# ChenyuWang-Monica/REED

Measured on AMD Instinct MI355X. Metric: SiT-XL/2 ImageNet-256 train images/sec, higher is better.
Workload: dtype bf16

## Files before the change

### include/reed_hip.h

```cpp
#ifndef REED_HIP_H
#define REED_HIP_H
#include <stdint.h>
#ifdef __cplusplus
extern "C" {
#endif

const char* reed_last_error(void);
int reed_version(void);
int reed_half_kind(void);

int reed_gemm(int layout, int epilogue, const void* P, int64_t ldp, const void* Q, int64_t ldq,
              int M, int N, int K, void* C, int64_t ldc, void* C2, int64_t ldc2, const void* R,
              int64_t ldr, const void* bias, const void* gate, int64_t ldgate, int rows_per_gate,
              float* dbias, int accumulate, int split_k, int64_t slab_stride, void* stream);

int reed_wgrad_group(int n, const void* const* dy, const void* const* x, float* const* dw, float* const* dbias,
                     const int* n_out, const int* k_in, int tokens, int accumulate, void* stream);
int reed_wgrad_group_deal(int n, const int* n_out, const int* k_in, const int* has_bias, int cus, unsigned* items);

int reed_set_cu_reserve(int n);
int reed_planning_cus(void);
int reed_set_concurrent_comm(int on);

int reed_gemm_force_tile(int tile);

int64_t reed_colsum_ws_floats(int M, int N);
int reed_colsum_bf16(const void* x, int64_t ld, float* ws, float* out, int M, int N, int accumulate,
                     void* stream);

int reed_reduce_slabs(const float* slabs, int64_t stride, int nslabs, float* out, int64_t n,
                      int accumulate, void* stream);

int reed_ln_modulate_fwd(const float* x, const void* shift, const void* scale, int64_t ldmod,
                         void* h, float* mean, float* rstd, int M, int D, int T, float eps,
                         void* stream);
int reed_ln_modulate_bwd(const void* dh, const float* x, const float* mean, const float* rstd,
                         const void* scale, int64_t ldmod, float* dx, float* part, int M, int D,
                         int T, void* stream);

int reed_ln_modulate_bwd_gate(const void* dh, const float* x, const float* mean, const float* rstd,
                              const void* scale, int64_t ldmod, float* dx, float* part, const void* y,
                              const void* gate, int64_t ldgate, void* dy, float* part_g, float* part_dy,
                              int M, int D, int T, void* stream);

int reed_gate_bwd(const float* dx, const void* y, const void* gate, int64_t ldgate, void* dy,
                  float* part, float* part_dy, int M, int D, int T, void* stream);
int reed_transpose_bf16(const void* src, void* dst, int R, int C, void* stream);
int reed_rowsum_f32(const float* part, int R, float* ws, float* out, int N, int accumulate, void* stream);

int reed_reduce_mod_parts(const float* const* parts, const int64_t* strides, const int64_t* offs,
                          int nparts, void* dmod, int64_t lddmod, int B, int D, int chunks,
                          void* stream);

int reed_attention_fwd(const void* qkv, void* o, float* lse, int B, int T, int H, int hd,
                       void* stream);
int reed_attention_bwd(const void* qkv, const void* o, const void* d_o, const float* lse,
                       void* dqkv, int B, int T, int H, int hd, void* stream);
int64_t reed_attention_bwd_ws_floats(int B, int T, int H);
int reed_attention_bwd_ws(const void* qkv, const void* o, const void* d_o, const float* lse, void* dqkv, float* ws,
                          int B, int T, int H, int hd, void* stream);
int reed_attention_bwd_dp(const void* qkv, const void* d_o, const float* lse, const float* dpart, void* dqkv, float* ws,
                          int B, int T, int H, int hd, void* stream);

int reed_qk_norm_fwd(const void* qkv, const float* qw, const float* qb, const float* kw, const float* kb,
                     void* out, float* stats, int M, int H, int hd, float eps, void* stream);
int64_t reed_qk_norm_bwd_part_floats(int M, int H, int hd);
int reed_qk_norm_bwd(const void* dn, const void* qkv, const float* stats, const float* qw, const float* kw,
                     void* dpre, float* part, int M, int H, int hd, void* stream);

int reed_patch_embed_fwd(const float* x, const void* w, const void* bias, const float* pos,
                         float* tokens, int B, int C, int HW, int P, int D, void* stream);
int reed_patchify_bf16(const float* x, void* out, int B, int C, int HW, int P, int order, void* stream);
int64_t reed_smallk_wgrad_ws_floats(int Dw, int KS);
int reed_smallk_wgrad(const void* wide, int wide_is_f32, const void* small, float* ws, float* out,
                      float* colsum_wide, float* colsum_small, int M, int Dw, int KS, int layout,
                      int accumulate, void* stream);
int reed_timestep_sinusoid(const float* t, void* out, int B, int dim, float max_period, void* stream);
int reed_label_cond(const int64_t* labels, const uint8_t* drop, int num_classes, int table_rows, const float* table,
                    const void* t_emb, int64_t* labels_out, float* c, void* silu_c, int* err_flag, int B, int D,
                    void* stream);
int reed_label_cond_bwd(const float* dsilu_c, const float* c, const int64_t* labels_eff, void* dt_emb,
                        float* dtable, int B, int D, void* stream);
int reed_final_layer_fwd(const float* x, const void* shift, const void* scale, int64_t ldmod,
                         const void* w, const void* bias, float* out, float* mean, float* rstd,
                         int B, int T, int D, int C, int P, float eps, void* stream);
int reed_final_layer_bwd_rows(const float* dout, const float* x, const float* mean, const float* rstd,
                              const void* shift, const void* scale, int64_t ldmod, const void* w,
                              void* hbuf, void* dlin, void* dh, int B, int T, int D, int C, int P,
                              void* stream);
int reed_token_mean_fwd(const float* x, void* out, int B, int T, int D, void* stream);
int reed_token_mean_bwd(const void* dmean, float* dx, int B, int T, int D, void* stream);

int reed_sample_posterior(const float* moments, const float* eps, float* out, int B, int64_t half,
                          float scale, float bias, void* stream);
int reed_interpolant(const float* x, const float* noise, const float* t, float* xt, float* target,
                     int B, int64_t per, int path_type, void* stream);
int reed_mse_fwd(const float* out, const float* target, float* loss, int B, int64_t per, void* stream);
int reed_mse_bwd(const float* out, const float* target, const float* gscale, float* dout, int B,
                 int64_t per, void* stream);
int reed_cosine_fwd(const void* zt, const float* z, float* rowdot, float* loss, int B, int T, int Z,
                    void* stream);
int reed_cosine_bwd(const void* zt, const float* z, const float* gscale, void* dzt, int B, int T,
                    int Z, void* stream);

int reed_grad_sqnorm(const float* g, int64_t n, float* partial, int nblocks, void* stream);
int reed_clip_finalize(const float* partial, int nblocks, float max_norm, float* norm_clip, void* stream);
int reed_clip_finalize_scaled(const float* partial, int nblocks, float max_norm, float* norm_clip, float* scaler_state,
                              float growth_factor, float backoff_factor, float growth_interval, void* stream);
int reed_adamw_ema(float* p, const float* g, float* m, float* v, float* ema, void* shadow,
                   int64_t n_train, int64_t n_total, const float* norm_clip, const float* scaler_state, float lr,
                   float beta1, float beta2, float eps, float weight_decay, float bc1, float bc2, float ema_decay,
                   void* stream);
int reed_cast_bf16(const float* src, void* dst, int64_t n, void* stream);

int reed_sampler_update(const double* x_cur, const float* model_out, const double* d_prev,
                        double* d_store, double* x_next, int64_t n_elems, int cfg, double cfg_scale,
                        double dt, double w0, double w1, void* stream);
int reed_sde_update(const double* x_cur, const float* model_out, const double* eps, double* x_next,
// ... 48 lines not shown
```

### reed_amd/csrc/norm.hip

```cpp
#include "../../include/reed_hip.h"
#include "common.hpp"

namespace {

constexpr int MAXV = 5;

__device__ __forceinline__ f32x4 ld_bf4(const bf16* p) {
  bf16x4 v = *(const bf16x4*)p;
  return f32x4{bf2f(v[0]), bf2f(v[1]), bf2f(v[2]), bf2f(v[3])};
}
__device__ __forceinline__ void st_bf4(bf16* p, f32x4 v) {
  bf16x4 o;
#pragma unroll
  for (int j = 0; j < 4; ++j) o[j] = f2bf(v[j]);
  *(bf16x4*)p = o;
}

template <bool NT>
__global__ __launch_bounds__(256) void ln_mod_fwd_kernel(const float* __restrict__ x, const bf16* __restrict__ shift,
                                                         const bf16* __restrict__ scale, long ldmod,
                                                         bf16* __restrict__ h, float* __restrict__ mean,
                                                         float* __restrict__ rstd, int M, int D, int T, float eps) {
  const int row = blockIdx.x * 4 + (threadIdx.x >> 6);
  if (row >= M) return;
  const int lane = threadIdx.x & 63, nv = D >> 2;
  const float* xr = x + (long)row * D;
  f32x4 v[MAXV];
  float s = 0.f;
#pragma unroll
  for (int k = 0; k < MAXV; ++k) {
    int idx = lane + 64 * k;
    const bool ok = idx < nv;
    if constexpr (NT) v[k] = __builtin_nontemporal_load((const f32x4*)(xr + (ok ? idx : 0) * 4));
    else v[k] = *(const f32x4*)(xr + (ok ? idx : 0) * 4);
    const float m = ok ? 1.f : 0.f;
    v[k] *= m;
    s += v[k][0] + v[k][1] + v[k][2] + v[k][3];
  }
  bf16* hr = h + (long)row * D;
  if (scale == nullptr) {
#pragma unroll
    for (int k = 0; k < MAXV; ++k) {
      int idx = lane + 64 * k;
      if (idx < nv) st_bf4(hr + idx * 4, v[k]);
    }
    return;
  }
  const float mu = wave_sum(s) / D;
  float q = 0.f;
#pragma unroll
  for (int k = 0; k < MAXV; ++k) {
    int idx = lane + 64 * k;
    if (idx < nv) {
#pragma unroll
      for (int j = 0; j < 4; ++j) { float d = v[k][j] - mu; q += d * d; }
    }
  }
  const float r = rsqrtf(wave_sum(q) / D + eps);
  if (lane == 0 && mean) { mean[row] = mu; rstd[row] = r; }
  const bf16* sc = scale + (long)(row / T) * ldmod;
  const bf16* sh = shift + (long)(row / T) * ldmod;
  f32x4 av[MAXV], bv[MAXV];
#pragma unroll
  for (int k = 0; k < MAXV; ++k) {
    int idx = lane + 64 * k;
    int ic = idx < nv ? idx : 0;
    av[k] = ld_bf4(sc + ic * 4);
    bv[k] = ld_bf4(sh + ic * 4);
  }
#pragma unroll
  for (int k = 0; k < MAXV; ++k) {
    int idx = lane + 64 * k;
    if (idx < nv) {
      f32x4 o;
#pragma unroll
      for (int j = 0; j < 4; ++j) o[j] = (v[k][j] - mu) * r * bfround(1.f + av[k][j]) + bv[k][j];
      st_bf4(hr + idx * 4, o);
    }
  }
}

template <bool GATE>
__global__ __launch_bounds__(256) void ln_mod_bwd_kernel(const bf16* __restrict__ dh, const float* __restrict__ x,
                                                         const float* __restrict__ mean, const float* __restrict__ rstd,
                                                         const bf16* __restrict__ scale, long ldmod,
                                                         float* __restrict__ dx, float* __restrict__ part,
                                                         const bf16* __restrict__ y, const bf16* __restrict__ gate,
                                                         long ldgate, bf16* __restrict__ dy, float* __restrict__ part_g,
                                                         float* __restrict__ part_dy, int M, int D, int T) {
  extern __shared__ __attribute__((aligned(16))) float red[];
  const int wave = threadIdx.x >> 6, lane = threadIdx.x & 63, nv = D >> 2;
  const int row0 = blockIdx.x * 16 + wave * 4;
  const long smp = (blockIdx.x * 16) / T;
  const bf16* sc = scale + smp * ldmod;
  f32x4 s1[MAXV], ps[MAXV], pq[MAXV];
  f32x4 gv[GATE ? MAXV : 1], pg[GATE ? MAXV : 1], pd[GATE ? MAXV : 1];
#pragma unroll
  for (int k = 0; k < MAXV; ++k) {
    int idx = lane + 64 * k;
    ps[k] = f32x4{0, 0, 0, 0};
    pq[k] = f32x4{0, 0, 0, 0};
    if (GATE) { pg[k] = f32x4{0, 0, 0, 0}; pd[k] = f32x4{0, 0, 0, 0}; }
    if (idx < nv) {
      f32x4 a = ld_bf4(sc + idx * 4);
#pragma unroll
      for (int j = 0; j < 4; ++j) s1[k][j] = bfround(1.f + a[j]);
      if (GATE) gv[k] = ld_bf4(gate + smp * ldgate + idx * 4);
    }
  }
  for (int rr = 0; rr < 4; ++rr) {
    const int row = row0 + rr;
    if (row >= M) break;
    const float mu = mean[row], r = rstd[row];
    f32x4 xh[MAXV], gy[MAXV], xin[MAXV], gin[MAXV];
    float a1 = 0.f, a2 = 0.f;
#pragma unroll
    for (int k = 0; k < MAXV; ++k) {
      int idx = lane + 64 * k;
      int ic = idx < nv ? idx : 0;
      xin[k] = *(const f32x4*)(x + (long)row * D + ic * 4);
      gin[k] = ld_bf4(dh + (long)row * D + ic * 4);
    }
#pragma unroll
    for (int k = 0; k < MAXV; ++k) {
      int idx = lane + 64 * k;
      if (idx < nv) {
        f32x4 xv = xin[k];
        f32x4 g = gin[k];
#pragma unroll
        for (int j = 0; j < 4; ++j) {
          xh[k][j] = (xv[j] - mu) * r;
          gy[k][j] = g[j] * s1[k][j];
          a1 += gy[k][j];
          a2 += gy[k][j] * xh[k][j];
          ps[k][j] += g[j];
          pq[k][j] += g[j] * xh[k][j];
        }
      }
    }
    f32x4 dold[MAXV], yin[GATE ? MAXV : 1];
#pragma unroll
    for (int k = 0; k < MAXV; ++k) {
      int idx = lane + 64 * k;
      dold[k] = *(const f32x4*)(dx + (long)row * D + (idx < nv ? idx : 0) * 4);
      if (GATE) yin[k] = ld_bf4(y + (long)row * D + (idx < nv ? idx : 0) * 4);
    }
    a1 = wave_sum(a1) / D;
    a2 = wave_sum(a2) / D;
#pragma unroll
    for (int k = 0; k < MAXV; ++k) {
      int idx = lane + 64 * k;
      if (idx < nv) {
        float* dp = dx + (long)row * D + idx * 4;
        f32x4 o = dold[k];
#pragma unroll
        for (int j = 0; j < 4; ++j) o[j] += r * (gy[k][j] - a1 - xh[k][j] * a2);
        *(f32x4*)dp = o;
        if (GATE) {
          f32x4 oy;
#pragma unroll
// ... 395 lines not shown
                                                             int T, int D) {
  const int b = blockIdx.y, d = blockIdx.x * 256 + threadIdx.x;
  if (d >= D) return;
  const float g = bf2f(dmean[(long)b * D + d]) / T;
  float* p = dx + (long)b * T * D + d;
  for (int t = 0; t < T; ++t) p[(long)t * D] += g;
}

__global__ __launch_bounds__(256) void cast_bf16_kernel(const float* __restrict__ s, bf16* __restrict__ d, long n4,
                                                        long n) {
  long i = (long)blockIdx.x * 256 + threadIdx.x;
  const long stride = (long)gridDim.x * 256;
  for (; i < n4; i += stride) st_bf4(d + i * 4, *(const f32x4*)(s + i * 4));
  if (blockIdx.x == 0 && threadIdx.x < (n & 3)) {
    long k = (n4 << 2) + threadIdx.x;
    d[k] = f2bf(s[k]);
  }
}

__global__ __launch_bounds__(256) void colsum_partial_kernel(const bf16* __restrict__ x, long ld, float* __restrict__ part,
                                                             int M, int N) {
  const int col = (blockIdx.x * 256 + threadIdx.x) * 4;
  if (col >= N) return;
  const int r0 = blockIdx.y * 256;
  f32x4 s = {0, 0, 0, 0};
  const bf16* base = x + (long)r0 * ld + col;
  if (r0 + 256 <= M) {
#pragma unroll 1
    for (int rr = 0; rr < 256; rr += 8) {
      f32x4 v[8];
#pragma unroll
      for (int k = 0; k < 8; ++k) v[k] = ld_bf4(base + (long)(rr + k) * ld);
#pragma unroll
      for (int k = 0; k < 8; ++k) s += v[k];
    }
  } else {
    for (int r = r0; r < M; ++r) s += ld_bf4(x + (long)r * ld + col);
  }
  *(f32x4*)(part + (long)blockIdx.y * N + col) = s;
}
__global__ __launch_bounds__(256) void colsum_reduce_kernel(const float* __restrict__ part, int nsl, float* __restrict__ out,
                                                            int N, int accumulate) {
  __shared__ float red[4][64];
  const int col = blockIdx.x * 64 + (threadIdx.x & 63), grp = threadIdx.x >> 6;
  float s = 0.f;
  if (col < N)
    for (int z = grp; z < nsl; z += 4) s += part[(long)z * N + col];
  red[grp][threadIdx.x & 63] = s;
  __syncthreads();
  if (grp == 0 && col < N) {
    float t = (red[0][threadIdx.x] + red[1][threadIdx.x]) + (red[2][threadIdx.x] + red[3][threadIdx.x]);
    out[col] = accumulate ? out[col] + t : t;
  }
}

__global__ __launch_bounds__(256) void reduce_slabs_kernel(const float* __restrict__ slabs, long stride, int ns,
                                                           float* __restrict__ out, long n, int accumulate) {
  long i = (long)blockIdx.x * 256 + threadIdx.x;
  if (i >= n) return;
  float s = accumulate ? out[i] : 0.f;
  for (int z = 0; z < ns; ++z) s += slabs[(long)z * stride + i];
  out[i] = s;
}

}

extern "C" int reed_ln_modulate_fwd(const float* x, const void* shift, const void* scale, int64_t ldmod,
                                    void* h, float* mean, float* rstd, int M, int D, int T, float eps,
                                    void* stream) {
  REED_CHECK_ARG(x && h, "ln_modulate_fwd: null pointer");
  REED_CHECK_ARG(D % 4 == 0 && D <= 256 * MAXV, "ln_modulate: D=%d unsupported (multiple of 4, <= %d)", D, 256 * MAXV);
  REED_CHECK_ARG(M > 0 && T > 0, "ln_modulate: bad M=%d T=%d", M, T);
  REED_CHECK_ARG((scale == nullptr) == (shift == nullptr), "ln_modulate: shift and scale must both be given or both NULL");
  if ((long)M * D * 4 >= (256l << 20))
    REED_KLAUNCH(ln_mod_fwd_kernel<true>, dim3(cdiv(M, 4)), dim3(256), 0, (hipStream_t)stream, x, (const bf16*)shift,
                 (const bf16*)scale, (long)ldmod, (bf16*)h, mean, rstd, M, D, T, eps);
  else
    REED_KLAUNCH(ln_mod_fwd_kernel<false>, dim3(cdiv(M, 4)), dim3(256), 0, (hipStream_t)stream, x, (const bf16*)shift,
                 (const bf16*)scale, (long)ldmod, (bf16*)h, mean, rstd, M, D, T, eps);
  REED_LAUNCH_CHECK();
  return REED_OK;
}

extern "C" int reed_ln_modulate_bwd(const void* dh, const float* x, const float* mean, const float* rstd,
                                    const void* scale, int64_t ldmod, float* dx, float* part, int M, int D,
                                    int T, void* stream) {
  REED_CHECK_ARG(dh && x && mean && rstd && scale && dx && part, "ln_modulate_bwd: null pointer");
  REED_CHECK_ARG(D % 4 == 0 && D <= 256 * MAXV, "ln_modulate: D=%d unsupported", D);
  REED_CHECK_ARG(T % 16 == 0 && M % 16 == 0, "ln_modulate_bwd: T=%d, M=%d must be multiples of 16", T, M);
  if (launch_ln_mod_bwd2<false>((hipStream_t)stream, (const bf16*)dh, x, mean, rstd, (const bf16*)scale, (long)ldmod, dx,
                                part, nullptr, nullptr, 0l, nullptr, nullptr, nullptr, M, D, T)) {
    REED_LAUNCH_CHECK();
    return REED_OK;
  }
    REED_KLAUNCH(ln_mod_bwd_kernel<false>, dim3(M / 16), dim3(256), 8 * D * sizeof(float), (hipStream_t)stream,
                 (const bf16*)dh, x, mean, rstd, (const bf16*)scale, (long)ldmod, dx, part, (const bf16*)nullptr,
                 (const bf16*)nullptr, 0l, (bf16*)nullptr, (float*)nullptr, (float*)nullptr, M, D, T);
  REED_LAUNCH_CHECK();
  return REED_OK;
}

extern "C" int reed_ln_modulate_bwd_gate(const void* dh, const float* x, const float* mean, const float* rstd,
                                         const void* scale, int64_t ldmod, float* dx, float* part, const void* y,
                                         const void* gate, int64_t ldgate, void* dy, float* part_g, float* part_dy,
                                         int M, int D, int T, void* stream) {
  REED_CHECK_ARG(dh && x && mean && rstd && scale && dx && part, "ln_modulate_bwd_gate: null pointer");
  REED_CHECK_ARG(y && gate && dy && part_g, "ln_modulate_bwd_gate: null gate operand");
  REED_CHECK_ARG(D % 4 == 0 && D <= 256 * MAXV, "ln_modulate: D=%d unsupported", D);
  REED_CHECK_ARG(T % 16 == 0 && M % 16 == 0, "ln_modulate_bwd_gate: T=%d, M=%d must be multiples of 16", T, M);
  if (launch_ln_mod_bwd2<true>((hipStream_t)stream, (const bf16*)dh, x, mean, rstd, (const bf16*)scale, (long)ldmod, dx,
                               part, (const bf16*)y, (const bf16*)gate, (long)ldgate, (bf16*)dy, part_g, part_dy, M, D, T)) {
    REED_LAUNCH_CHECK();
    return REED_OK;
  }
    REED_KLAUNCH(ln_mod_bwd_kernel<true>, dim3(M / 16), dim3(256), 8 * D * sizeof(float), (hipStream_t)stream,
                 (const bf16*)dh, x, mean, rstd, (const bf16*)scale, (long)ldmod, dx, part, (const bf16*)y,
                 (const bf16*)gate, (long)ldgate, (bf16*)dy, part_g, part_dy, M, D, T);
  REED_LAUNCH_CHECK();
  return REED_OK;
}

extern "C" int reed_transpose_bf16(const void* src, void* dst, int R, int C, void* stream) {
  REED_CHECK_ARG(src && dst && R > 0 && C > 0, "transpose_bf16: bad args");
  if (R % 64 == 0 && C % 64 == 0 && ((uintptr_t)src % 8) == 0 && ((uintptr_t)dst % 8) == 0)
    REED_KLAUNCH(transpose_bf16_v4_kernel, dim3(C / 64, R / 64), dim3(256), 0, (hipStream_t)stream, (const bf16*)src, (bf16*)dst, R, C);
  else
    REED_KLAUNCH(transpose_bf16_kernel, dim3(cdiv(C, 64), cdiv(R, 64)), dim3(256), 0, (hipStream_t)stream,
                 (const bf16*)src, (bf16*)dst, R, C);
  REED_LAUNCH_CHECK();
  return REED_OK;
}

__global__ __launch_bounds__(256) void rowsum_stage1_kernel(const float* __restrict__ part, int R, float* __restrict__ part2,
                                                            int N) {
  const int col = blockIdx.x * 256 + threadIdx.x;
  if (col >= N) return;
  const int r0 = blockIdx.y * 64, r1 = min(R, r0 + 64);
  float s = 0.f;
  int r = r0;
  for (; r + 8 <= r1; r += 8) {
    float v[8];
#pragma unroll
    for (int k = 0; k < 8; ++k) v[k] = part[(long)(r + k) * N + col];
#pragma unroll
    for (int k = 0; k < 8; ++k) s += v[k];
  }
  for (; r < r1; ++r) s += part[(long)r * N + col];
  part2[(long)blockIdx.y * N + col] = s;
}

extern "C" int reed_rowsum_f32(const float* part, int R, float* ws, float* out, int N, int accumulate, void* stream) {
  REED_CHECK_ARG(part && out && R > 0 && N > 0, "rowsum_f32: bad args");
  if (R > 256 && ws) {
    const int R2 = cdiv(R, 64);
    REED_KLAUNCH(rowsum_stage1_kernel, dim3(cdiv(N, 256), R2), dim3(256), 0, (hipStream_t)stream, part, R, ws, N);
    REED_KLAUNCH(rowsum_f32_kernel, dim3(cdiv(N, 64)), dim3(256), 0, (hipStream_t)stream, ws, R2, out, N, accumulate);
  } else {
    REED_KLAUNCH(rowsum_f32_kernel, dim3(cdiv(N, 64)), dim3(256), 0, (hipStream_t)stream, part, R, out, N, accumulate);
  }
  REED_LAUNCH_CHECK();
  return REED_OK;
}

extern "C" int reed_gate_bwd(const float* dx, const void* y, const void* gate, int64_t ldgate, void* dy,
                             float* part, float* part_dy, int M, int D, int T, void* stream) {
  REED_CHECK_ARG(dx && y && gate && dy && part, "gate_bwd: null pointer");
// ... 76 lines not shown
```

### reed_amd/engine.py

```python
import contextlib
import os
import types

import torch

from . import ops
from .ops import (NT, NN, TN, EPI_BF16, EPI_GELU, EPI_SILU, EPI_GATE_RES, EPI_DGELU, EPI_DSILU, EPI_F32, EPI_ADDF32_RB,
                  EPI_GELU_G, EPI_SILU_G, EPI_MUL)


class Engine:
    DGRAD_NT_MIN_TOKENS = 12289
    SAVE_ACT_GRAD_MIN_TOKENS = 12288
    WGRAD_STREAM_MAX_TOKENS = 0

    def __init__(self, model):
        self.m = model
        self.L = model._layout
        self.A = model._arena
        if self.A.master.device.type != "cuda":
            raise RuntimeError("reed_amd.SiT: parameters are on %s; move the model to an AMD GPU (model.cuda()). "
                               "The hot path has no CPU fallback." % self.A.master.device)
        self.D = model.hidden_size
        self.H = model.num_heads
        self.hd = self.D // self.H
        self.Hm = int(self.D * model.mlp_ratio)
        self.T = model.num_patches
        self.P = model.patch_size
        self.C = model.in_channels
        self.depth = model.depth
        self.NO = self.P * self.P * self.C
        self._dims_ok = set()
        split = model.encoder_depth_text is not None and model.encoder_depth_text != model.encoder_depth
        self.split = split
        self.tap_depth = [model.encoder_depth if (zt == "i" or not split) else model.encoder_depth_text
                          for zt in model.z_types]
        self.reducer = None
        self._dot_delta = {}
        self._ws = None
        self._named = None
        self._sentinel = None
        self._ws_side = None
        self._shadow_t = None
        self.dgrad_nt = None
        self.split_ada_wgrad = None
        self._side = None
        self.wgrad_stream = {"0": False, "1": True}.get(os.environ.get("REED_WGRAD_STREAM", "auto"))
        self.wgrad_stream_max_tokens = self.WGRAD_STREAM_MAX_TOKENS
        self.grad_live = False
        self.table_rows = model.num_classes + (1 if model.class_dropout_prob > 0 else 0)
        self._hb = 2
        self.save_act_grad = None
        self.fused_delta = True
        self._err = None

    def _check_dims(self, prec):
        if prec in self._dims_ok:
            return
        q = 4 if prec == "fp32" else 128
        what = "4 (fp32 operands)" if prec == "fp32" else "128 for the MFMA GEMM tiles"
        for n, v in (("hidden_size", self.D), ("mlp hidden", self.Hm), ("projector_dim", self.m.projector_dim)):
            if v % q:
                raise ValueError(f"{n}={v} must be a multiple of {what}")
        for z in self.m.z_dims:
            if z % q:
                raise ValueError(f"z_dim={z} must be a multiple of {what}")
        self._dims_ok.add(prec)

    def check_errors(self):
        if self._err is not None and int(self._err.item()) != 0:
            self._err.zero_()
            raise IndexError(f"reed_amd.SiT: a class label outside [0, {self.table_rows}) was passed to the model "
                             f"(num_classes={self.m.num_classes}, class_dropout_prob={self.m.class_dropout_prob}); "
                             "the affected forwards used row 0 instead")

    def W(self, name):
        return self._shadow.data_ptr() + self._hb * self.L.off(name)

    def Wf(self, name):
        return self.A.master.data_ptr() + 4 * self.L.off(name)

    def G(self, name):
        return self.A.grad.data_ptr() + 4 * self.L.off(name)

    def ws(self, nfloats, dev):
        if self._ws is None or self._ws.numel() < nfloats:
            self._ws = torch.empty(int(nfloats), dtype=torch.float32, device=dev)
        return self._ws

    def ws_side(self, nfloats, dev):
        if self._ws_side is None or self._ws_side.numel() < nfloats:
            self._ws_side = torch.empty(int(nfloats), dtype=torch.float32, device=dev)
        return self._ws_side

    def forward(self, x, t, y, inference, need_grad, drop):
        prec = getattr(self.m, "precision", "bf16")
        prev = ops.use(prec)
        try:
            return self._forward(x, t, y, inference, need_grad, drop, prec)
        finally:
            ops.use(prev)

    def _forward(self, x, t, y, inference, need_grad, drop, prec):
        m, L = self.m, self.L
        ops.require_cuda(x, "x")
        dev = x.device
        B, C, HW = x.shape[0], x.shape[1], x.shape[-1]
        D, H, hd, Hm, T, P = self.D, self.H, self.hd, self.Hm, self.T, self.P
        if C != self.C or HW != m.input_size or x.shape[-2] != HW:
            raise ValueError(f"input {tuple(x.shape)} does not match (N,{self.C},{m.input_size},{m.input_size})")
        M = B * T
        self._check_dims(prec)
        self._shadow = self.A.ensure_shadow(prec)
        hdt = ops.half_dtype(prec)
        hb = self._hb = hdt.itemsize
        pend = self.A.pending
        if "all" in pend:
            self.A.wait_all()
        elif pend:
            self.A.wait("embed")
        x = x.contiguous().float()
        t = t.contiguous().float()
        y = y.contiguous().long()

        def bf(*s):
            return torch.empty(s, dtype=hdt, device=dev)

        def f32(*s):
            return torch.empty(s, dtype=torch.float32, device=dev)

        sag = self.save_act_grad if self.save_act_grad is not None else M > self.SAVE_ACT_GRAD_MIN_TOKENS
        self._sag = sag
        tp = types.SimpleNamespace(B=B, blocks=[], proj={}, x=x, prec=prec, act_grad=sag) if need_grad else None
        epi_silu = EPI_SILU_G if need_grad and sag else EPI_SILU
        epi_gelu = EPI_GELU_G if need_grad and sag else EPI_GELU
        tok = f32(M, D)
        ops.patch_embed_fwd(x, self.W("x_embedder.proj.weight"), self.W("x_embedder.proj.bias"), self.Wf("pos_embed"),
                            tok, B, C, HW, P, D)
        sin = bf(B, 256)
        ops.timestep_sinusoid(t, sin, B)
        t1p = bf(B, D) if need_grad else None
        t1 = bf(B, D)
        ops.gemm(NT, epi_silu, sin, self.W("t_embedder.mlp.0.weight"), B, D, 256, t1p, 256, 256, D, C2=t1, ldc2=D,
                 bias=self.W("t_embedder.mlp.0.bias"))
        temb = bf(B, D)
        ops.gemm(NT, EPI_BF16, t1, self.W("t_embedder.mlp.2.weight"), B, D, D, temb, D, D, D,
                 bias=self.W("t_embedder.mlp.2.bias"))
        drop_u8 = None
        if drop is not None:
            drop_u8 = drop.to(device=dev, dtype=torch.uint8).contiguous()
        labels_eff = torch.empty(B, dtype=torch.int64, device=dev)
        c = f32(B, D)
        silu_c = bf(B, D)
        if self._err is None:
            self._err = torch.zeros(1, dtype=torch.int32, device=dev)
        ops.label_cond(y, drop_u8, m.num_classes, self.Wf("y_embedder.embedding_table.weight"), temb, labels_eff, c,
                       silu_c, B, D, table_rows=self.table_rows, err=self._err)
        Nall = L.ada_rows
        mod = bf(B, Nall)
        sp = self._shadow.data_ptr()
        mp = mod.data_ptr()
        kh = min(L.ADA_HEAD_BLOCKS, self.depth) if "ada_tail" in pend else 0
        n_head = kh * 6 * D if kh else Nall
        if pend:
            self.A.wait("ada_head")
        ops.gemm(NT, EPI_BF16, silu_c, sp + hb * L.ada_w_off, B, n_head, D, mod, D, D, Nall, bias=sp + hb * L.ada_b_off)
        if need_grad:
            tp.sin, tp.t1p, tp.t1, tp.labels_eff, tp.c, tp.silu_c, tp.mod = sin, t1p, t1, labels_eff, c, silu_c, mod

        if not need_grad:
            xa, xb = tok, f32(M, D)
            h, qkv, o, u = bf(M, D), bf(M, 3 * D), bf(M, D), bf(M, Hm)
        xcur = tok
        zs_by_proj = {}
        for i in range(self.depth):
            b = f"blocks.{i}."
            mb = mp + hb * (i * 6 * D)
            if kh and i == kh:
                self.A.wait("ada_tail")
                ops.gemm(NT, EPI_BF16, silu_c, sp + hb * (L.ada_w_off + n_head * D), B, Nall - n_head, D, mp + hb * n_head,
                         D, D, Nall, bias=sp + hb * (L.ada_b_off + n_head))
                kh = 0
            if pend:
                self.A.wait(f"block{i}")
            if need_grad:
                h, qkv, o, u = bf(M, D), bf(M, 3 * D), bf(M, D), bf(M, Hm)
                h2, a1, y1, y2 = bf(M, D), bf(M, Hm), bf(M, D), bf(M, D)
                mean1, rstd1, mean2, rstd2 = f32(M), f32(M), f32(M), f32(M)
                lse = f32(B, H, T)
                xmid, xout = f32(M, D), f32(M, D)
            else:
                h2, a1, y1, y2 = h, None, None, None
                mean1 = rstd1 = mean2 = rstd2 = lse = None
                xmid = xb if xcur is xa else xa
                xout = xcur
            ops.ln_modulate_fwd(xcur, mb, mb + hb * D, Nall, h, mean1, rstd1, M, D, T)
            ops.gemm(NT, EPI_BF16, h, self.W(b + "attn.qkv.weight"), M, 3 * D, D, qkv, D, D, 3 * D,
                     bias=self.W(b + "attn.qkv.bias"))
            qkv_a, qstats = qkv, None
            if m.qk_norm:
                qkv_a = bf(M, 3 * D)
                qstats = f32(M, 2, H, 2) if need_grad else None
                ops.qk_norm_fwd(qkv, self.Wf(b + "attn.q_norm.weight"), self.Wf(b + "attn.q_norm.bias"),
                                self.Wf(b + "attn.k_norm.weight"), self.Wf(b + "attn.k_norm.bias"), qkv_a, qstats, M, H, hd)
            ops.attention_fwd(qkv_a, o, lse, B, T, H, hd)
            ops.gemm(NT, EPI_GATE_RES, o, self.W(b + "attn.proj.weight"), M, D, D, xmid, D, D, D, C2=y1, ldc2=D,
                     R=xcur, ldr=D, bias=self.W(b + "attn.proj.bias"), gate=mb + 2 * hb * D, ldgate=Nall, rows_per_gate=T)
            ops.ln_modulate_fwd(xmid, mb + 3 * hb * D, mb + 4 * hb * D, Nall, h2, mean2, rstd2, M, D, T)
            ops.gemm(NT, epi_gelu, h2, self.W(b + "mlp.fc1.weight"), M, Hm, D, a1, D, D, Hm, C2=u, ldc2=Hm,
                     bias=self.W(b + "mlp.fc1.bias"))
            ops.gemm(NT, EPI_GATE_RES, u, self.W(b + "mlp.fc2.weight"), M, D, Hm, xout, Hm, Hm, D, C2=y2, ldc2=D,
                     R=xmid, ldr=D, bias=self.W(b + "mlp.fc2.bias"), gate=mb + 5 * hb * D, ldgate=Nall, rows_per_gate=T)
            if need_grad:
                tp.blocks.append(types.SimpleNamespace(x=xcur, mean1=mean1, rstd1=rstd1, h=h, qkv=qkv, qkv_a=qkv_a,
                                                       qstats=qstats, o=o, lse=lse,
                                                       y1=y1, xmid=xmid, mean2=mean2, rstd2=rstd2, h2=h2, a1=a1, u=u,
                                                       y2=y2))
            xcur = xout
            if not inference:
                for j, dj in enumerate(self.tap_depth):
                    if dj == i + 1:
                        zs_by_proj[j] = self._projector_fwd(j, xcur, B, need_grad, tp)
        if kh:
            self.A.wait("ada_tail")
            ops.gemm(NT, EPI_BF16, silu_c, sp + hb * (L.ada_w_off + n_head * D), B, Nall - n_head, D, mp + hb * n_head,
                     D, D, Nall, bias=sp + hb * (L.ada_b_off + n_head))
        if pend:
            self.A.wait_all()
        out = f32(B, C, HW, HW)
        meanF = f32(M) if need_grad else None
        rstdF = f32(M) if need_grad else None
        mf = mp + hb * (self.depth * 6 * D)
        ops.final_layer_fwd(xcur, mf, mf + hb * D, Nall, self.W("final_layer.linear.weight"),
                            self.W("final_layer.linear.bias"), out, meanF, rstdF, B, T, D, C, P)
        if need_grad:
            tp.x_last, tp.meanF, tp.rstdF = xcur, meanF, rstdF
        zs = None
        if not inference:
            if self.split:
                ji, jt = m.z_types.index("i"), m.z_types.index("t")
                zs = [zs_by_proj[ji], zs_by_proj[jt]]
                if need_grad:
                    tp.zs_order = [ji, jt]
            else:
                zs = [zs_by_proj[j] for j in range(len(m.z_dims))]
                if need_grad:
                    tp.zs_order = list(range(len(m.z_dims)))
        return out, zs, tp

    def _projector_fwd(self, j, x, B, need_grad, tp):
        m, D, T = self.m, self.D, self.T
        Pd, Z = m.projector_dim, m.z_dims[j]
        dev = x.device
        img = m.z_types[j] == "i"
        self.A.wait("projectors")
        R = B * T if img else B
        hdt = ops.half_dtype()
        bf = lambda *s: torch.empty(s, dtype=hdt, device=dev)
        xin = bf(R, D)
        if img:
            ops.ln_modulate_fwd(x, None, None, 0, xin, None, None, R, D, T)
        else:
            ops.token_mean_fwd(x, xin, B, T, D)
        pre = f"projectors.{j}."
        epi_silu = EPI_SILU_G if need_grad and self._sag else EPI_SILU
        p1p, p1 = (bf(R, Pd) if need_grad else None), bf(R, Pd)
        ops.gemm(NT, epi_silu, xin, self.W(pre + "0.weight"), R, Pd, D, p1p, D, D, Pd, C2=p1, ldc2=Pd,
                 bias=self.W(pre + "0.bias"))
        p2p, p2 = (bf(R, Pd) if need_grad else None), bf(R, Pd)
        ops.gemm(NT, epi_silu, p1, self.W(pre + "2.weight"), R, Pd, Pd, p2p, Pd, Pd, Pd, C2=p2, ldc2=Pd,
                 bias=self.W(pre + "2.bias"))
        zt = bf(R, Z)
        ops.gemm(NT, EPI_BF16, p2, self.W(pre + "4.weight"), R, Z, Pd, zt, Pd, Pd, Z, bias=self.W(pre + "4.bias"))
        if need_grad:
            tp.proj[j] = types.SimpleNamespace(xin=xin, p1p=p1p, p1=p1, p2p=p2p, p2=p2, R=R)
        return zt.view(B, T, Z) if img else zt

    def _wgrad_block(self, probs, Mtok, acc, dev, side):
        args = [(dy, x, self.G(w), self.G(w.replace("weight", "bias")), N, K) for dy, x, w, N, K in probs]
        if side is not None:
            side.wait_stream(torch.cuda.current_stream())
        with torch.cuda.stream(side) if side is not None else contextlib.nullcontext():
            done = ops.wgrad_group(args, Mtok, accumulate=acc)
        if not done:
            for dy, x, w, N, K in probs:
                self._wgrad(dy, x, w, Mtok, N, K, acc, dev, side=side)
            return
        if side is not None:
            for dy, x, _, _, _ in probs:
                dy.record_stream(side)
                x.record_stream(side)

    def _wgrad(self, dy, x, wname, Mtok, N, K, acc, dev, bias_done=False, side=None):
        bname = wname.replace("weight", "bias")
        lay, split = ops.plan_wgrad(Mtok, N, K)
# ... 377 lines not shown
```

### reed_amd/ops.py

```python
import ctypes

import math

import torch

from . import _lib

NT, NN, TN = 0, 1, 2
TN_TALL, TN_WIDE = 3, 4
(EPI_BF16, EPI_GELU, EPI_SILU, EPI_GATE_RES, EPI_DGELU, EPI_DSILU, EPI_F32, EPI_ADDF32_RB, EPI_ATOMIC_F32, EPI_QGELU,
 EPI_RES_BF16, EPI_GELU_ERF, EPI_LS_RES, EPI_BF16_DOT, EPI_GELU_G, EPI_SILU_G, EPI_MUL, EPI_SWIGLU) = range(18)
SWIGLU_GROUP = 8


def _p(t):
    if t is None:
        return None
    if isinstance(t, int):
        return t
    return t.data_ptr()


def _stream():
    return torch._C._cuda_getCurrentRawStream(torch._C._cuda_getDevice())
# ... 215 lines not shown
def wgrad_group_deal(shapes, cus=256, precision="bf16"):
    n = len(shapes)
    ip = ctypes.c_int * n
    items = (ctypes.c_uint * 256)()
    L = _lib.load(precision)
    T = L.reed_wgrad_group_deal(n, ctypes.cast(ip(*[int(q[0]) for q in shapes]), ctypes.c_void_p),
                                ctypes.cast(ip(*[int(q[1]) for q in shapes]), ctypes.c_void_p),
                                ctypes.cast(ip(*[int(bool(q[2])) for q in shapes]), ctypes.c_void_p), int(cus),
                                ctypes.cast(items, ctypes.c_void_p))
    if T <= 0:
        return None
    wpx, out = cus // 8, []
    for x in range(8):
        run = []
        for j in range(wpx):
            it = items[x * wpx + j]
            if it == 0xFFFFFFFF:
                continue
            mode, mu, nu = (it >> 2) & 15, (it >> 6) & 255, (it >> 14) & 255
            vm, vn = ((it >> 22) & 3) + 1, ((it >> 24) & 3) + 1
            rows = {0: 256, 6: 128 * vm, 7: 128, 8: 128 * vm}[mode]
            cols = {0: 256, 6: 128, 7: 128 * vn, 8: 0}[mode]
            run.append(dict(p=it & 3, mode=mode, row=128 * mu, col=128 * nu, rows=rows, cols=cols, bias=(it >> 26) & 1))
        out.append(run)
    assert sum(len(r) for r in out) == T
    return out


def wgrad_group(problems, tokens, accumulate=False):
    n = len(problems)
    vp, ip = ctypes.c_void_p * n, ctypes.c_int * n
    dy = vp(*[_p(q[0]) for q in problems])
    x = vp(*[_p(q[1]) for q in problems])
    dw = vp(*[_p(q[2]) for q in problems])
    db = vp(*[_p(q[3]) for q in problems])
    no = ip(*[int(q[4]) for q in problems])
    ki = ip(*[int(q[5]) for q in problems])
    cast = lambda a: ctypes.cast(a, ctypes.c_void_p)
    L = _lib.load(_PRECISION)
    key = wgrad_group_probe(tokens, [(int(q[4]), int(q[5])) for q in problems]) if wgrad_group_probe is not None else None
    if key is not None:
        e0, e1 = torch.cuda.Event(enable_timing=True), torch.cuda.Event(enable_timing=True)
        e0.record()
    rc = L.reed_wgrad_group(n, cast(dy), cast(x), cast(dw), cast(db), cast(no), cast(ki), int(tokens), int(accumulate),
                            _stream())
    if rc == 1002:
        return False
    _lib.check(rc, "reed_wgrad_group", L)
    if key is not None:
        e1.record()
        gemm_probe_log.append((key, e0, e1))
    return True


def plan_wgrad(Mtok, N, K):
    ktiles = (Mtok + 63) // 64
    slots = wgrad_slots()
    best, best_key = (TN, 1), None
    for lay, bm, bn, rate in WGRAD_TILES:
        if K % bn or N % 128:
            continue
        tiles = ((N + bm - 1) // bm) * (K // bn)
        fill = (N * K) / (tiles * bm * bn)
        for s in range(1, WGRAD_SPLIT_MAX + 1):
            if s > 1 and ktiles // s < 32:
                break
            blocks = tiles * s
            eff = blocks / (((blocks + slots - 1) // slots) * slots)
            dist = abs(math.log((ktiles / s) / 256.0))
            key = (-round(rate * fill * eff / 0.03), dist)
            if best_key is None or key < best_key:
                best, best_key = (lay, s), key
    return best


def reduce_slabs(slabs, stride, n, out, count, accumulate=False):
    _call("reed_reduce_slabs", _p(slabs), stride, n, _p(out), count, int(accumulate), _stream())


def ln_modulate_fwd(x, shift, scale, ldmod, h, mean, rstd, M, D, T, eps=1e-6):
    _call("reed_ln_modulate_fwd", _p(x), _p(shift), _p(scale), ldmod, _p(h), _p(mean), _p(rstd), M, D, T, eps, _stream())


def ln_modulate_bwd(dh, x, mean, rstd, scale, ldmod, dx, part, M, D, T):
    _call("reed_ln_modulate_bwd", _p(dh), _p(x), _p(mean), _p(rstd), _p(scale), ldmod, _p(dx), _p(part), M, D, T, _stream())


def ln_modulate_bwd_gate(dh, x, mean, rstd, scale, ldmod, dx, part, y, gate, ldgate, dy, part_g, part_dy, M, D, T):
    _call("reed_ln_modulate_bwd_gate", _p(dh), _p(x), _p(mean), _p(rstd), _p(scale), ldmod, _p(dx), _p(part), _p(y),
          _p(gate), ldgate, _p(dy), _p(part_g), _p(part_dy), M, D, T, _stream())


def gate_bwd(dx, y, gate, ldgate, dy, part, M, D, T, part_dy=None):
    _call("reed_gate_bwd", _p(dx), _p(y), _p(gate), ldgate, _p(dy), _p(part), _p(part_dy), M, D, T, _stream())


def transpose_bf16(src, dst, R, C):
    _call("reed_transpose_bf16", _p(src), _p(dst), R, C, _stream())


def rowsum_f32(part, R, out, N, accumulate=False, ws=None):
    _call("reed_rowsum_f32", _p(part), R, _p(ws), _p(out), N, int(accumulate), _stream())


def reduce_mod_parts(parts, dmod, lddmod, B, D, chunks):
    n = len(parts)
    ptrs = (ctypes.c_void_p * n)(*[_p(p[0]) for p in parts])
    strides = (ctypes.c_int64 * n)(*[p[1] for p in parts])
    offs = (ctypes.c_int64 * n)(*[p[2] for p in parts])
    _call("reed_reduce_mod_parts", ptrs, strides, offs, n, _p(dmod), lddmod, B, D, chunks, _stream())


def token_mean_fwd(x, out, B, T, D):
    _call("reed_token_mean_fwd", _p(x), _p(out), B, T, D, _stream())


def token_mean_bwd(dmean, dx, B, T, D):
    _call("reed_token_mean_bwd", _p(dmean), _p(dx), B, T, D, _stream())


def cast_bf16(src, dst, n):
    _call("reed_cast_bf16", _p(src), _p(dst), n, _stream())


def attention_fwd(qkv, o, lse, B, T, H, hd):
    _call("reed_attention_fwd", _p(qkv), _p(o), _p(lse), B, T, H, hd, _stream())


def attention_bwd(qkv, o, do, lse, dqkv, B, T, H, hd, ws=None):
    if ws is None:
        _call("reed_attention_bwd", _p(qkv), _p(o), _p(do), _p(lse), _p(dqkv), B, T, H, hd, _stream())
    else:
        _call("reed_attention_bwd_ws", _p(qkv), _p(o), _p(do), _p(lse), _p(dqkv), _p(ws), B, T, H, hd, _stream())


def attention_bwd_dp(qkv, do, lse, dpart, dqkv, ws, B, T, H, hd):
    _call("reed_attention_bwd_dp", _p(qkv), _p(do), _p(lse), _p(dpart), _p(dqkv), _p(ws), B, T, H, hd, _stream())


def dgrad_with_head_dots(dy, w, dx, o, dpart, M, N, K, hd, wt=None):
    L = _lib.load(_PRECISION)
    if wt is not None:
        rc = L.reed_gemm(NT, EPI_BF16_DOT, _p(dy), N, _p(wt), N, M, K, N, _p(dx), K, _p(dpart), 0, _p(o), K, None, None, 0, hd, None, 0,
                         1, 0, _stream())
    else:
        rc = L.reed_gemm(NN, EPI_BF16_DOT, _p(dy), N, _p(w), K, M, K, N, _p(dx), K, _p(dpart), 0, _p(o), K, None, None, 0, hd, None, 0,
                         1, 0, _stream())
    if rc == 1002:
        return False
    _lib.check(rc, "reed_gemm", L)
    return True


def attention_bwd_ws_floats(B, T, H):
    return int(_lib.load(_PRECISION).reed_attention_bwd_ws_floats(B, T, H))


def qk_norm_fwd(qkv, qw, qb, kw, kb, out, stats, M, H, hd, eps=1e-5):
    _call("reed_qk_norm_fwd", _p(qkv), _p(qw), _p(qb), _p(kw), _p(kb), _p(out), _p(stats), M, H, hd, eps, _stream())


def qk_norm_part_floats(M, H, hd):
    return int(_lib.load().reed_qk_norm_bwd_part_floats(M, H, hd))


def qk_norm_bwd(dn, qkv, stats, qw, kw, dpre, part, M, H, hd):
# ... 168 lines not shown
```

Measured before the change: 1323.

## Move gated residual out of GEMM epilogue into fused residual+LN-modulate kernel

Adds a row-wise kernel that applies the gated residual (x + gate*y), writes the fp32 residual stream, and in the same pass computes LayerNorm statistics and the adaLN-modulated bf16 output for the next consumer. The forward block now runs attn.proj and fc2 GEMMs with a plain bf16 epilogue, then this fused kernel, and carries the next block's LN output across iterations. This removes a separate LN pass that re-read the fp32 residual and moves the heavier gate/residual epilogue out of the GEMM. In exchange the GEMM writes y to memory and the new kernel reads it back. The ada_tail GEMM is also scheduled one block earlier to supply the next block's modulation.

```diff
diff --git a/include/reed_hip.h b/include/reed_hip.h
--- a/include/reed_hip.h
+++ b/include/reed_hip.h
@@ -34,6 +34,9 @@
 int reed_ln_modulate_fwd(const float* x, const void* shift, const void* scale, int64_t ldmod,
                          void* h, float* mean, float* rstd, int M, int D, int T, float eps,
                          void* stream);
+int reed_gate_res_ln_modulate_fwd(const void* y, const void* gate, int64_t ldgate, const float* x_in, float* x_out,
+                                  const void* shift, const void* scale, int64_t ldmod, void* h, float* mean,
+                                  float* rstd, int M, int D, int T, float eps, void* stream);
 int reed_ln_modulate_bwd(const void* dh, const float* x, const float* mean, const float* rstd,
                          const void* scale, int64_t ldmod, float* dx, float* part, int M, int D,
                          int T, void* stream);
diff --git a/reed_amd/csrc/norm.hip b/reed_amd/csrc/norm.hip
--- a/reed_amd/csrc/norm.hip
+++ b/reed_amd/csrc/norm.hip
@@ -76,6 +76,84 @@
 #pragma unroll
       for (int j = 0; j < 4; ++j) o[j] = (v[k][j] - mu) * r * bfround(1.f + av[k][j]) + bv[k][j];
       st_bf4(hr + idx * 4, o);
+    }
+  }
+}
+
+template <bool NT, bool LN>
+__global__ __launch_bounds__(256) void gate_res_ln_mod_fwd_kernel(const bf16* __restrict__ y, const bf16* __restrict__ gate,
+                                                                  long ldgate, const float* x_in, float* x_out,
+                                                                  const bf16* __restrict__ shift, const bf16* __restrict__ scale,
+                                                                  long ldmod, bf16* __restrict__ h, float* __restrict__ mean,
+                                                                  float* __restrict__ rstd, int M, int D, int T, float eps) {
+  const int row = blockIdx.x * 4 + (threadIdx.x >> 6);
+  if (row >= M) return;
+  const int lane = threadIdx.x & 63, nv = D >> 2;
+  const float* xr = x_in + (long)row * D;
+  const bf16* yr = y + (long)row * D;
+  const bf16* gr = gate + (long)(row / T) * ldgate;
+  f32x4 v[MAXV], yv[MAXV], gv[MAXV];
+#pragma unroll
+  for (int k = 0; k < MAXV; ++k) {
+    int idx = lane + 64 * k;
+    int ic = idx < nv ? idx : 0;
+    if constexpr (NT) v[k] = __builtin_nontemporal_load((const f32x4*)(xr + ic * 4));
+    else v[k] = *(const f32x4*)(xr + ic * 4);
+    if constexpr (NT) {
+      const bf16x4 t = __builtin_nontemporal_load((const bf16x4*)(yr + ic * 4));
+      yv[k] = f32x4{bf2f(t[0]), bf2f(t[1]), bf2f(t[2]), bf2f(t[3])};
+    } else yv[k] = ld_bf4(yr + ic * 4);
+    gv[k] = ld_bf4(gr + ic * 4);
+  }
+  float* xo = x_out + (long)row * D;
+  float s = 0.f;
+#pragma unroll
+  for (int k = 0; k < MAXV; ++k) {
+    int idx = lane + 64 * k;
+    const bool ok = idx < nv;
+#pragma unroll
+    for (int j = 0; j < 4; ++j) v[k][j] = v[k][j] + bfround(gv[k][j] * yv[k][j]);
+    if (ok) {
+      if constexpr (NT) __builtin_nontemporal_store(v[k], (f32x4*)(xo + idx * 4));
+      else *(f32x4*)(xo + idx * 4) = v[k];
+    }
+    const float m = ok ? 1.f : 0.f;
+    v[k] *= m;
+    s += v[k][0] + v[k][1] + v[k][2] + v[k][3];
+  }
+  if constexpr (LN) {
+    const float mu = wave_sum(s) / D;
+    float q = 0.f;
+#pragma unroll
+    for (int k = 0; k < MAXV; ++k) {
+      int idx = lane + 64 * k;
+      if (idx < nv) {
+#pragma unroll
+        for (int j = 0; j < 4; ++j) { float d = v[k][j] - mu; q += d * d; }
+      }
+    }
+    const float r = rsqrtf(wave_sum(q) / D + eps);
+    if (lane == 0 && mean) { mean[row] = mu; rstd[row] = r; }
+    const bf16* sc = scale + (long)(row / T) * ldmod;
+    const bf16* sh = shift + (long)(row / T) * ldmod;
+    bf16* hr = h + (long)row * D;
+    f32x4 av[MAXV], bv[MAXV];
+#pragma unroll
+    for (int k = 0; k < MAXV; ++k) {
+      int idx = lane + 64 * k;
+      int ic = idx < nv ? idx : 0;
+      av[k] = ld_bf4(sc + ic * 4);
+      bv[k] = ld_bf4(sh + ic * 4);
+    }
+#pragma unroll
+    for (int k = 0; k < MAXV; ++k) {
+      int idx = lane + 64 * k;
+      if (idx < nv) {
+        f32x4 o;
+#pragma unroll
+        for (int j = 0; j < 4; ++j) o[j] = (v[k][j] - mu) * r * bfround(1.f + av[k][j]) + bv[k][j];
+        st_bf4(hr + idx * 4, o);
+      }
     }
   }
 }
@@ -637,6 +715,33 @@
   return REED_OK;
 }
 
+extern "C" int reed_gate_res_ln_modulate_fwd(const void* y, const void* gate, int64_t ldgate, const float* x_in, float* x_out,
+                                             const void* shift, const void* scale, int64_t ldmod, void* h, float* mean,
+                                             float* rstd, int M, int D, int T, float eps, void* stream) {
+  REED_CHECK_ARG(y && gate && x_in && x_out, "gate_res_ln_modulate_fwd: null pointer");
+  REED_CHECK_ARG(D % 4 == 0 && D <= 256 * MAXV, "gate_res_ln_modulate: D=%d unsupported (multiple of 4, <= %d)", D, 256 * MAXV);
+  REED_CHECK_ARG(M > 0 && T > 0, "gate_res_ln_modulate: bad M=%d T=%d", M, T);
+  REED_CHECK_ARG((h == nullptr) == (scale == nullptr) && (h == nullptr) == (shift == nullptr),
+                 "gate_res_ln_modulate: h, shift and scale must all be given or all NULL (the residual alone)");
+  REED_CHECK_ARG((mean == nullptr) == (rstd == nullptr) && (h || !mean),
+                 "gate_res_ln_modulate: mean and rstd come together, and only with h");
+  const bool nt = (long)M * D * 4 >= (256l << 20);
+#define REED_GRL(NT_, LN_)                                                                                                   \
+  REED_KLAUNCH((gate_res_ln_mod_fwd_kernel<NT_, LN_>), dim3(cdiv(M, 4)), dim3(256), 0, (hipStream_t)stream, (const bf16*)y, \
+               (const bf16*)gate, (long)ldgate, x_in, x_out, (const bf16*)shift, (const bf16*)scale, (long)ldmod, (bf16*)h,  \
+               mean, rstd, M, D, T, eps)
+  if (h) {
+    if (nt) REED_GRL(true, true);
+    else REED_GRL(false, true);
+  } else {
+    if (nt) REED_GRL(true, false);
+    else REED_GRL(false, false);
+  }
+#undef REED_GRL
+  REED_LAUNCH_CHECK();
+  return REED_OK;
+}
+
 extern "C" int reed_ln_modulate_bwd(const void* dh, const float* x, const float* mean, const float* rstd,
                                     const void* scale, int64_t ldmod, float* dx, float* part, int M, int D,
                                     int T, void* stream) {
diff --git a/reed_amd/engine.py b/reed_amd/engine.py
--- a/reed_amd/engine.py
+++ b/reed_amd/engine.py
@@ -13,6 +13,7 @@
     DGRAD_NT_MIN_TOKENS = 12289
     SAVE_ACT_GRAD_MIN_TOKENS = 12288
     WGRAD_STREAM_MAX_TOKENS = 0
+    GATE_RES_ROWS_MIN_TOKENS = 0
 
     def __init__(self, model):
         self.m = model
@@ -43,6 +44,7 @@
         self._ws_side = None
         self._shadow_t = None
         self.dgrad_nt = None
+        self.gate_res_rows = None
         self.split_ada_wgrad = None
         self._side = None
         self.wgrad_stream = {"0": False, "1": True}.get(os.environ.get("REED_WGRAD_STREAM", "auto"))
@@ -168,15 +170,18 @@
         if need_grad:
             tp.sin, tp.t1p, tp.t1, tp.labels_eff, tp.c, tp.silu_c, tp.mod = sin, t1p, t1, labels_eff, c, silu_c, mod
 
+        rows = self.gate_res_rows if self.gate_res_rows is not None else M >= self.GATE_RES_ROWS_MIN_TOKENS
         if not need_grad:
             xa, xb = tok, f32(M, D)
             h, qkv, o, u = bf(M, D), bf(M, 3 * D), bf(M, D), bf(M, Hm)
+            ys = bf(M, D) if rows else None
         xcur = tok
         zs_by_proj = {}
+        nxt = None
         for i in range(self.depth):
             b = f"blocks.{i}."
             mb = mp + hb * (i * 6 * D)
-            if kh and i == kh:
+            if kh and (i == kh or (rows and i + 1 == kh)):
                 self.A.wait("ada_tail")
                 ops.gemm(NT, EPI_BF16, silu_c, sp + hb * (L.ada_w_off + n_head * D), B, Nall - n_head, D, mp + hb * n_head,
                          D, D, Nall, bias=sp + hb * (L.ada_b_off + n_head))
@@ -184,17 +189,19 @@
             if pend:
                 self.A.wait(f"block{i}")
             if need_grad:
-                h, qkv, o, u = bf(M, D), bf(M, 3 * D), bf(M, D), bf(M, Hm)
+                qkv, o, u = bf(M, 3 * D), bf(M, D), bf(M, Hm)
+                h, mean1, rstd1 = nxt if nxt is not None else (bf(M, D), f32(M), f32(M))
                 h2, a1, y1, y2 = bf(M, D), bf(M, Hm), bf(M, D), bf(M, D)
-                mean1, rstd1, mean2, rstd2 = f32(M), f32(M), f32(M), f32(M)
+                mean2, rstd2 = f32(M), f32(M)
                 lse = f32(B, H, T)
                 xmid, xout = f32(M, D), f32(M, D)
             else:
-                h2, a1, y1, y2 = h, None, None, None
+                h2, a1, y1, y2 = h, None, ys, ys
                 mean1 = rstd1 = mean2 = rstd2 = lse = None
                 xmid = xb if xcur is xa else xa
                 xout = xcur
-            ops.ln_modulate_fwd(xcur, mb, mb + hb * D, Nall, h, mean1, rstd1, M, D, T)
+            if nxt is None:
+                ops.ln_modulate_fwd(xcur, mb, mb + hb * D, Nall, h, mean1, rstd1, M, D, T)
             ops.gemm(NT, EPI_BF16, h, self.W(b + "attn.qkv.weight"), M, 3 * D, D, qkv, D, D, 3 * D,
                      bias=self.W(b + "attn.qkv.bias"))
             qkv_a, qstats = qkv, None
@@ -204,13 +211,27 @@
                 ops.qk_norm_fwd(qkv, self.Wf(b + "attn.q_norm.weight"), self.Wf(b + "attn.q_norm.bias"),
                                 self.Wf(b + "attn.k_norm.weight"), self.Wf(b + "attn.k_norm.bias"), qkv_a, qstats, M, H, hd)
             ops.attention_fwd(qkv_a, o, lse, B, T, H, hd)
-            ops.gemm(NT, EPI_GATE_RES, o, self.W(b + "attn.proj.weight"), M, D, D, xmid, D, D, D, C2=y1, ldc2=D,
-                     R=xcur, ldr=D, bias=self.W(b + "attn.proj.bias"), gate=mb + 2 * hb * D, ldgate=Nall, rows_per_gate=T)
-            ops.ln_modulate_fwd(xmid, mb + 3 * hb * D, mb + 4 * hb * D, Nall, h2, mean2, rstd2, M, D, T)
+            if rows:
+                ops.gemm(NT, EPI_BF16, o, self.W(b + "attn.proj.weight"), M, D, D, y1, D, D, D, bias=self.W(b + "attn.proj.bias"))
+                ops.gate_res_ln_modulate_fwd(y1, mb + 2 * hb * D, Nall, xcur, xmid, mb + 3 * hb * D, mb + 4 * hb * D, Nall, h2,
+                                             mean2, rstd2, M, D, T)
+            else:
+                ops.gemm(NT, EPI_GATE_RES, o, self.W(b + "attn.proj.weight"), M, D, D, xmid, D, D, D, C2=y1, ldc2=D,
+                         R=xcur, ldr=D, bias=self.W(b + "attn.proj.bias"), gate=mb + 2 * hb * D, ldgate=Nall, rows_per_gate=T)
+                ops.ln_modulate_fwd(xmid, mb + 3 * hb * D, mb + 4 * hb * D, Nall, h2, mean2, rstd2, M, D, T)
             ops.gemm(NT, epi_gelu, h2, self.W(b + "mlp.fc1.weight"), M, Hm, D, a1, D, D, Hm, C2=u, ldc2=Hm,
                      bias=self.W(b + "mlp.fc1.bias"))
-            ops.gemm(NT, EPI_GATE_RES, u, self.W(b + "mlp.fc2.weight"), M, D, Hm, xout, Hm, Hm, D, C2=y2, ldc2=D,
-                     R=xmid, ldr=D, bias=self.W(b + "mlp.fc2.bias"), gate=mb + 5 * hb * D, ldgate=Nall, rows_per_gate=T)
+            if rows:
+                ops.gemm(NT, EPI_BF16, u, self.W(b + "mlp.fc2.weight"), M, D, Hm, y2, Hm, Hm, D, bias=self.W(b + "mlp.fc2.bias"))
+                if i + 1 < self.depth:
+                    nxt = (bf(M, D), f32(M), f32(M)) if need_grad else (h, None, None)
+                    mn = mb + hb * 6 * D
+                    ops.gate_res_ln_modulate_fwd(y2, mb + 5 * hb * D, Nall, xmid, xout, mn, mn + hb * D, Nall, *nxt, M, D, T)
+                else:
+                    ops.gate_res_ln_modulate_fwd(y2, mb + 5 * hb * D, Nall, xmid, xout, None, None, 0, None, None, None, M, D, T)
+            else:
+                ops.gemm(NT, EPI_GATE_RES, u, self.W(b + "mlp.fc2.weight"), M, D, Hm, xout, Hm, Hm, D, C2=y2, ldc2=D,
+                         R=xmid, ldr=D, bias=self.W(b + "mlp.fc2.bias"), gate=mb + 5 * hb * D, ldgate=Nall, rows_per_gate=T)
             if need_grad:
                 tp.blocks.append(types.SimpleNamespace(x=xcur, mean1=mean1, rstd1=rstd1, h=h, qkv=qkv, qkv_a=qkv_a,
                                                        qstats=qstats, o=o, lse=lse,
diff --git a/reed_amd/ops.py b/reed_amd/ops.py
--- a/reed_amd/ops.py
+++ b/reed_amd/ops.py
@@ -321,6 +321,11 @@
     _call("reed_ln_modulate_fwd", _p(x), _p(shift), _p(scale), ldmod, _p(h), _p(mean), _p(rstd), M, D, T, eps, _stream())
 
 
+def gate_res_ln_modulate_fwd(y, gate, ldgate, x_in, x_out, shift, scale, ldmod, h, mean, rstd, M, D, T, eps=1e-6):
+    _call("reed_gate_res_ln_modulate_fwd", _p(y), _p(gate), ldgate, _p(x_in), _p(x_out), _p(shift), _p(scale), ldmod, _p(h),
+          _p(mean), _p(rstd), M, D, T, eps, _stream())
+
+
 def ln_modulate_bwd(dh, x, mean, rstd, scale, ldmod, dx, part, M, D, T):
     _call("reed_ln_modulate_bwd", _p(dh), _p(x), _p(mean), _p(rstd), _p(scale), ldmod, _p(dx), _p(part), M, D, T, _stream())
 
```

New measurement: 1328 (median of 6 runs). About the same (+0.4%).
